# JingruiYu/FishBirdEyeVisualSLAM

Hardware: AMD Instinct MI355X
Metric: frames/s (extract+match+pose-opt), 1280x720+512x512 pair (higher is better)
Workload: dtype u8 (extract, Hamming) + f64 (pose optimisation); 1 GPU; configs[2]: 1280x720 front + 512x512 bird pair, HIP ORB extract + M3/M9 Hamming match + PoseOptimizationWithBird (~2k front + ~1k bird edges); nfeatures=2000, parallelism=replicas x1

## Files before the change

fishbirdeyevisualslam_amd/csrc/orb.hip:

```cpp
#include "fb_common.h"
#include "fb_fast_score.h"
#include "fb_primitives.h"

namespace {

constexpr int EDGE_THRESHOLD = 19;
constexpr int HALF_PATCH = 15;
constexpr int PATCH_SIZE = 31;
constexpr int BORDER = EDGE_THRESHOLD - 3;

__constant__ float c_pattern[1024] = {
#include "orb_pattern.inc"
};

struct LevelInfo {
  int w, h, pitch;
  long long off;
  int nCols, nRows, wCell, hCell, cellBase;
  int N;
  long long candBase;
  int candCap;
  int slotCap;
  int outBase, outCap;
  int nIni;
  float hX;
  float scale;
  int patchSize;
  long long boff;
};

struct OrbK {
  int nlevels, iniTh, minTh, totalCells, outStride, capOut;
  int kpStride;
  int fastTileBytes, fastMaxOut, fastMaxPix;
  int fastTP;
  int dbg;
  unsigned long long *timers;
  int cellBase[FB_MAX_LEVELS + 1];
  int grpBase[FB_MAX_LEVELS + 1];
  int totalGroups;
  long long pyrStride;
  long long blurStride;
  int blurStrips[FB_MAX_LEVELS + 1];
  long long candStride;
  int umax[16];
  LevelInfo L[FB_MAX_LEVELS];
};

struct ResizeTabs {
  const int *xofs;
  const short *ialpha;
  const int *yofs;
  const short *ibeta;
};

__device__ __forceinline__ int win_byte(uint32_t w0, uint32_t w1, uint32_t w2, uint32_t w3, int k) {
  const uint32_t lo = k & 8 ? w2 : w0, hi = k & 8 ? w3 : w1;
  const uint32_t w = k & 4 ? hi : lo;
  return (w >> (8 * (k & 3))) & 0xFF;
}

__global__ __launch_bounds__(256) void k_resize(const uint8_t *__restrict__ src0, long long srcImgStride, int sw,
                                                int sh, int spitch, uint8_t *__restrict__ dst0, long long dstImgStride,
                                                int dw, int dh, int dpitch, ResizeTabs tb) {
  const int b = blockIdx.z;
  const int dy = blockIdx.y * blockDim.y + threadIdx.y;
  const int dx4 = (blockIdx.x * blockDim.x + threadIdx.x) * 4;
  if (dy >= dh || dx4 >= dpitch) return;
  const uint8_t *src = src0 + (long long)b * srcImgStride;
  uint8_t *dst = dst0 + (long long)b * dstImgStride;
  int sy0 = tb.yofs[dy], sy1 = sy0 + 1;
  sy0 = sy0 >= 0 ? (sy0 < sh ? sy0 : sh - 1) : 0;
  sy1 = sy1 >= 0 ? (sy1 < sh ? sy1 : sh - 1) : 0;
  const int b0 = tb.ibeta[dy * 2], b1 = tb.ibeta[dy * 2 + 1];
  const uint8_t *r0p = src + (long long)sy0 * spitch, *r1p = src + (long long)sy1 * spitch;
  uint32_t packed = 0;
  const int dxl = min(dx4 + 3, dw - 1);
  const int sxa = dx4 < dw ? tb.xofs[dx4] : 0, sxb = dx4 < dw ? min(tb.xofs[dxl] + 1, sw - 1) : 0;
  const int a = sxa & ~3;
  const bool wide = ((reinterpret_cast<uintptr_t>(src) | (uintptr_t)spitch) & 3) == 0 && (sxb - a) < 16 && a + 16 <= spitch;
  if (wide) {
    const uint32_t *p0 = reinterpret_cast<const uint32_t *>(r0p + a), *p1 = reinterpret_cast<const uint32_t *>(r1p + a);
    const uint32_t u0 = p0[0], u1 = p0[1], u2 = p0[2], u3 = p0[3], v0 = p1[0], v1 = p1[1], v2 = p1[2], v3 = p1[3];
#pragma unroll
    for (int k = 0; k < 4; k++) {
// ... 504 lines not shown
          int oq = o - TP - 1;
          asm volatile("" : "+v"(oq));
          const uint8_t *q = &sc[oq] + TP + 1;
          const int sv = q[0];
          if (sv >= Tk) {
            const int mx = max(max(max(max((int)q[-1], (int)q[1]), (int)q[-tp - 1]), max((int)q[-tp], (int)q[-tp + 1])),
                               max(max((int)q[tp - 1], (int)q[tp]), (int)q[tp + 1]));
            keep = sv > mx;
            const int yy = o / tp, xx = o - yy * tp - ox;
            rec = (uint32_t)(x0 + xx) | ((uint32_t)(y0 + yy) << 12) | ((uint32_t)sv << 24);
          }
        }
        const unsigned long long m = __ballot(keep);
        if (keep) s_out[total + (int)__builtin_amdgcn_mbcnt_hi((uint32_t)(m >> 32), __builtin_amdgcn_mbcnt_lo((uint32_t)m, 0u))] = rec;
        total += __popcll(m);
      }
      if (pass == 0) { FAST_TICK(4) } else { FAST_TICK(7) }
      if (K.dbg == 3) { if (total == 12345) cand[0] = 1; return; }
      if (total == 0) continue;
      __syncthreads();
      uint32_t *out = cand + (long long)b * K.candStride + Lv.candBase + (long long)cell * Lv.slotCap;
#pragma unroll 1
      for (int i = lane; i < total; i += 64) out[i] = s_out[i];
      if (lane == 0) cellCount[(long long)b * K.totalCells + Lv.cellBase + cell] = total;
      if (pass == 0) { FAST_TICK(5) } else { FAST_TICK(8) }
      break;
    }
  };
  int ci = __builtin_amdgcn_readfirstlane(cFirst / Lv.nCols), cj = cFirst - ci * Lv.nCols;
  Geo g = geo(ci, cj);
  if (timed) { if (g.cw + g.ch + g.x0 + g.y0 == 123456789) cand[0] = 1; }
  FAST_TICK(9)
  if (g.ok && aligned) issue(g);
  for (int cell = cFirst; cell < cEnd; cell++) {
    const bool haveNext = cell + 1 < cEnd;
    if (haveNext) { cj++; if (cj == Lv.nCols) { cj = 0; ci++; } }
    const Geo gn = geo(ci, cj);
    if (g.ok) {
      stage(g);
      if (timed) { if (tile[lane] == 255 && sc[lane] == 7) cand[0] = 1; }
      FAST_TICK(0)
      __builtin_amdgcn_s_waitcnt(0x0F70);
      if (haveNext && gn.ok && aligned) issue(gn);
      FAST_TICK(1)
      process(g, cell);
      __syncthreads();
    } else if (haveNext && gn.ok && aligned) {
      issue(gn);
    }
    g = gn;
  }
  if (TIMED && timed && lane == 0) {
#pragma unroll
    for (int i = 0; i < 10; i++) atomicAdd(&K.timers[i], (unsigned long long)t_acc[i]);
    atomicAdd(&K.timers[10], (unsigned long long)(t_mark - t_start));
    atomicAdd(&K.timers[11], 1ull);
  }
#undef FAST_TICK
}

struct ONode {
  short x0, y0, x1, y1;
  int cnt;
};

__device__ __forceinline__ int quadrant(const ONode &n, int rx, int ry) {
  const int halfX = (int)ceilf((float)(n.x1 - n.x0) / 2), halfY = (int)ceilf((float)(n.y1 - n.y0) / 2);
  const int mx = n.x0 + halfX, my = n.y0 + halfY;
  return (rx < mx ? 0 : 1) + (ry < my ? 0 : 2);
}

__device__ __forceinline__ ONode child_of(const ONode &n, int q, int cnt) {
  const int halfX = (int)ceilf((float)(n.x1 - n.x0) / 2), halfY = (int)ceilf((float)(n.y1 - n.y0) / 2);
  const int mx = n.x0 + halfX, my = n.y0 + halfY;
  ONode c;
  c.x0 = (q & 1) ? mx : n.x0;
  c.x1 = (q & 1) ? n.x1 : mx;
  c.y0 = (q & 2) ? my : n.y0;
  c.y1 = (q & 2) ? n.y1 : my;
  c.cnt = cnt;
  return c;
}

template <int NT>
__global__ __launch_bounds__(NT) void k_octree(OrbK K, const uint32_t *__restrict__ cellCand, const int *__restrict__ cellCount,
                                                uint32_t *__restrict__ cand, int *__restrict__ candCount, uint16_t *__restrict__ nodeOf,
                                                uint32_t *__restrict__ lvlOut, int *__restrict__ lvlCount, int maxNodes) {
  extern __shared__ __attribute__((aligned(16))) uint8_t smem[];
  const int l = blockIdx.y, b = blockIdx.x, tid = threadIdx.x;
  const LevelInfo &Lv = K.L[l];
  const int M = maxNodes;
  ONode *listA = reinterpret_cast<ONode *>(smem);
  ONode *listB = listA + M;
  int *ccnt = reinterpret_cast<int *>(listB + M);
  unsigned short *cpos = reinterpret_cast<unsigned short *>(ccnt + 4 * M);
  unsigned short *npos = cpos + 4 * M;
  unsigned short *order = npos + M;
  unsigned char *split = reinterpret_cast<unsigned char *>(order + M);
  unsigned long long *best = reinterpret_cast<unsigned long long *>(smem + (((size_t)(split + M - smem)) + 7 & ~(size_t)7));
  __shared__ int s_w[NT / 64], s_S, s_nexp, s_jstar;
  uint32_t *cdw = cand + (long long)b * K.candStride + Lv.candBase;
  int n;
  {
    int *offs = reinterpret_cast<int *>(smem);
    const int ncell = Lv.nCols * Lv.nRows;
    const int *cc = cellCount + (long long)b * K.totalCells + Lv.cellBase;
    const uint32_t *sp = cellCand + (long long)b * K.candStride + Lv.candBase;
    int run = 0;
    for (int c0 = 0; c0 < ncell; c0 += NT) {
      const int c = c0 + tid;
      const int v = c < ncell ? cc[c] : 0;
      int tot;
      const int ex = fb::block_excl_scan<NT>(v, s_w, &tot);
      if (c < ncell) offs[c] = run + ex;
      run += tot;
      __syncthreads();
    }
    n = run;
    if (tid == 0) { offs[ncell] = n; candCount[b * K.nlevels + l] = n; }
    __syncthreads();
    for (int k0 = tid; k0 < n; k0 += NT * 4) {
      uint32_t val[4];
#pragma unroll
      for (int u = 0; u < 4; u++) {
        const int k = min(k0 + u * NT, n - 1);
        int lo = 0, hi = ncell;
        while (hi - lo > 1) {
          const int mid = (lo + hi) >> 1;
          if (offs[mid] <= k) lo = mid; else hi = mid;
        }
        val[u] = sp[(long long)lo * Lv.slotCap + (k - offs[lo])];
      }
#pragma unroll
      for (int u = 0; u < 4; u++)
        if (k0 + u * NT < n) cdw[k0 + u * NT] = val[u];
    }
    __threadfence_block();
    __syncthreads();
  }
  const uint32_t *cd = cdw;
  uint16_t *nof = nodeOf + (long long)b * K.candStride + Lv.candBase;
  int *outCount = lvlCount + b * K.nlevels + l;
  uint32_t *out = lvlOut + (long long)b * K.outStride + Lv.outBase;
  if (n == 0 || Lv.nIni < 1) { if (tid == 0) *outCount = 0; return; }
  const int N = Lv.N;
  const int Hh = Lv.h - 2 * BORDER;
  for (int i = tid; i < Lv.nIni; i += NT) {
    ONode nd;
    nd.x0 = (short)(int)(Lv.hX * (float)i);
    nd.x1 = (short)(int)(Lv.hX * (float)(i + 1));
    nd.y0 = 0; nd.y1 = (short)Hh; nd.cnt = 0;
    listB[i] = nd;
  }
  __syncthreads();
  for (int k = tid; k < n; k += NT) {
    const int rx = (int)(cd[k] & 0xFFF) - BORDER;
    int idx = (int)((float)rx / Lv.hX);
    idx = min(idx, Lv.nIni - 1);
    nof[k] = (uint16_t)idx;
    atomicAdd(&listB[idx].cnt, 1);
  }
  __syncthreads();
  if (tid == 0) {
    int S = 0;
    for (int i = 0; i < Lv.nIni; i++) {
      npos[i] = (unsigned short)S;
      if (listB[i].cnt > 0) listA[S++] = listB[i];
    }
    s_S = S;
  }
  __syncthreads();
  for (int k = tid; k < n; k += NT) nof[k] = npos[nof[k]];
  __syncthreads();
  ONode *cur = listA, *nxt = listB;
  int S = s_S;
  bool finalPhase = false;
  for (int guard = 0; guard < 64; guard++) {
    const int prevSize = S;
    for (int i = tid; i < 4 * S; i += NT) ccnt[i] = 0;
    __syncthreads();
    for (int k0 = tid; k0 < n; k0 += NT * 4) {
      int pk[4];
      uint32_t ck[4];
#pragma unroll
      for (int u = 0; u < 4; u++) { const int kk = min(k0 + u * NT, n - 1); pk[u] = nof[kk]; ck[u] = cd[kk]; }
#pragma unroll
      for (int u = 0; u < 4; u++) {
        if (k0 + u * NT >= n) break;
        const int p = pk[u];
        const ONode nd = cur[p];
        if (nd.cnt > 1) {
          const uint32_t c = ck[u];
          atomicAdd(&ccnt[4 * p + quadrant(nd, (int)(c & 0xFFF) - BORDER, (int)((c >> 12) & 0xFFF) - BORDER)], 1);
        }
      }
    }
    __syncthreads();
    if (!finalPhase) {
      for (int p = tid; p < S; p += NT) split[p] = cur[p].cnt > 1;
    } else {
      for (int p = tid; p < S; p += NT) {
        split[p] = 0;
        const int c = cur[p].cnt;
        if (c > 1) {
          int rank = 0;
          for (int j = 0; j < S; j++) {
            const int cj = cur[j].cnt;
            if (cj > 1 && (cj > c || (cj == c && j < p))) rank++;
          }
          order[rank] = (unsigned short)p;
        }
      }
      __syncthreads();
      if (tid == 0) {
        int sz = S, j = 0;
        const int C = s_nexp;
        for (; j < C; j++) {
          const int p = order[j];
          const int kk = (ccnt[4 * p] > 0) + (ccnt[4 * p + 1] > 0) + (ccnt[4 * p + 2] > 0) + (ccnt[4 * p + 3] > 0);
          sz += kk - 1;
          split[p] = 1;
          if (sz >= N) { j++; break; }
        }
        s_jstar = j;
      }
    }
    __syncthreads();
    const int per = (S + NT - 1) / NT;
    const int a0 = min(tid * per, S), a1 = min(a0 + per, S);
    int myKids = 0, myKeep = 0;
    if (!finalPhase) {
      for (int p = a0; p < a1; p++) {
        if (split[p]) myKids += (ccnt[4 * p] > 0) + (ccnt[4 * p + 1] > 0) + (ccnt[4 * p + 2] > 0) + (ccnt[4 * p + 3] > 0);
        else myKeep++;
      }
    } else {
      const int J = s_jstar;
      const int perj = (J + NT - 1) / NT;
      const int r0 = min(tid * perj, J), r1 = min(r0 + perj, J);
      for (int r = r0; r < r1; r++) {
        const int p = order[r];
        myKids += (ccnt[4 * p] > 0) + (ccnt[4 * p + 1] > 0) + (ccnt[4 * p + 2] > 0) + (ccnt[4 * p + 3] > 0);
      }
      for (int p = a0; p < a1; p++) if (!split[p]) myKeep++;
    }
    int totalKids, totalKeep;
    const int kidsBefore = fb::block_excl_scan<NT>(myKids, s_w, &totalKids);
    const int keepBefore = fb::block_excl_scan<NT>(myKeep, s_w, &totalKeep);
    {
      int ci = kidsBefore, kp = totalKids + keepBefore;
      if (!finalPhase) {
        for (int p = a0; p < a1; p++) {
          if (split[p]) {
            for (int q = 0; q < 4; q++)
              if (ccnt[4 * p + q] > 0) {
                const int pos = totalKids - 1 - ci++;
                cpos[4 * p + q] = (unsigned short)pos;
                nxt[pos] = child_of(cur[p], q, ccnt[4 * p + q]);
              }
          } else {
            npos[p] = (unsigned short)kp;
            nxt[kp++] = cur[p];
          }
        }
      } else {
        const int J = s_jstar;
        const int perj = (J + NT - 1) / NT;
        const int r0 = min(tid * perj, J), r1 = min(r0 + perj, J);
        for (int r = r0; r < r1; r++) {
          const int p = order[r];
          for (int q = 0; q < 4; q++)
            if (ccnt[4 * p + q] > 0) {
              const int pos = totalKids - 1 - ci++;
              cpos[4 * p + q] = (unsigned short)pos;
              nxt[pos] = child_of(cur[p], q, ccnt[4 * p + q]);
            }
        }
        for (int p = a0; p < a1; p++)
          if (!split[p]) { npos[p] = (unsigned short)kp; nxt[kp++] = cur[p]; }
      }
    }
    const int Snew = totalKids + totalKeep;
    __syncthreads();
    for (int k0 = tid; k0 < n; k0 += NT * 4) {
      int pk[4];
      uint32_t ck[4];
#pragma unroll
      for (int u = 0; u < 4; u++) { const int kk = min(k0 + u * NT, n - 1); pk[u] = nof[kk]; ck[u] = cd[kk]; }
#pragma unroll
      for (int u = 0; u < 4; u++) {
        const int k = k0 + u * NT;
        if (k >= n) break;
        const int p = pk[u];
        if (split[p]) {
          const uint32_t c = ck[u];
          nof[k] = cpos[4 * p + quadrant(cur[p], (int)(c & 0xFFF) - BORDER, (int)((c >> 12) & 0xFFF) - BORDER)];
        } else nof[k] = npos[p];
      }
    }
    int myExp = 0;
    {
      const int pern = (Snew + NT - 1) / NT;
      const int n0 = min(tid * pern, Snew), n1 = min(n0 + pern, Snew);
      for (int p = n0; p < n1; p++) myExp += (p < totalKids && nxt[p].cnt > 1);
    }
    int nToExpand;
    fb::block_excl_scan<NT>(myExp, s_w, &nToExpand);
    if (tid == 0) s_nexp = nToExpand;
    __syncthreads();
    ONode *t = cur; cur = nxt; nxt = t;
    S = Snew;
    if (S >= N || S == prevSize) break;
    if (!finalPhase) {
      if (S + nToExpand * 3 > N) finalPhase = true;
    }
  }
  for (int p = tid; p < S; p += NT) best[p] = 0ull;
  __syncthreads();
  for (int k0 = tid; k0 < n; k0 += NT * 4) {
    int pk[4];
    uint32_t ck[4];
#pragma unroll
    for (int u = 0; u < 4; u++) { const int kk = min(k0 + u * NT, n - 1); pk[u] = nof[kk]; ck[u] = cd[kk]; }
#pragma unroll
    for (int u = 0; u < 4; u++) {
    const int k = k0 + u * NT;
    if (k >= n) break;
    const uint32_t c = ck[u];
    const int x = c & 0xFFF, y = (c >> 12) & 0xFFF, r = c >> 24;
    const int cellI = (y - EDGE_THRESHOLD) / Lv.hCell, cellJ = (x - EDGE_THRESHOLD) / Lv.wCell;
    const int dwid = min(Lv.wCell, Lv.w - 2 * EDGE_THRESHOLD - cellJ * Lv.wCell);
    const int inCell = (y - EDGE_THRESHOLD - cellI * Lv.hCell) * dwid + (x - EDGE_THRESHOLD - cellJ * Lv.wCell);
    const unsigned orderKey = (unsigned)(cellI * Lv.nCols + cellJ) * 4096u + (unsigned)inCell;
    const unsigned long long key = ((unsigned long long)r << 56) | ((unsigned long long)(0xFFFFFFFFu - orderKey) << 24) | (unsigned)k;
    atomicMax(&best[pk[u]], key);
    }
  }
  __syncthreads();
  for (int p = tid; p < S; p += NT) out[p] = cd[(unsigned)(best[p] & 0xFFFFFFull)];
  if (tid == 0) *outCount = S;
}

constexpr int BLUR_ROWS = 32;

__device__ __forceinline__ int reflect101(int i, int n) {
  if (i < 0) i = -i;
  if (i >= n) i = 2 * n - 2 - i;
  return i;
}

__global__ __launch_bounds__(256) void k_blur(OrbK K, const uint8_t *__restrict__ img0, long long imgStride, int pitch0,
                                              const uint8_t *__restrict__ pyr, uint8_t *__restrict__ blur) {
  const int b = blockIdx.y;
  const int strip = __builtin_amdgcn_readfirstlane(blockIdx.x * 4 + (threadIdx.x >> 6));
  const int lane = threadIdx.x & 63;
  if (strip >= K.blurStrips[K.nlevels]) return;
  int l = 0;
  while (strip >= K.blurStrips[l + 1]) l++;
  const LevelInfo &L = K.L[l];
  const int w = L.w, h = L.h;
  const int sidx = strip - K.blurStrips[l];
  const int nsx = (w + 255) >> 8;
  const int sy = sidx / nsx, sx = sidx - sy * nsx;
  const int x0 = sx * 256 + lane * 4;
  const int y0 = sy * BLUR_ROWS;
  if (x0 >= w) return;
  const uint8_t *img;
  int pitch;
  if (l == 0) { img = img0 + (long long)b * imgStride; pitch = pitch0; }
  else { img = pyr + (long long)b * K.pyrStride + L.off; pitch = L.pitch; }
  uint8_t *out = blur + (long long)b * K.blurStride + L.boff;
  const bool edge = x0 < 4 || x0 + 8 > w;
  const int base = edge ? max(min(x0 - 4, w - 12), 0) : x0 - 4;
  uint32_t m1[3] = {0, 0, 0}, m2[3] = {0, 0, 0};
  if (edge) {
#pragma unroll
    for (int i = 0; i < 12; i++) {
      const int c = reflect101(min(x0 - 4 + i, w + 2), w);
      const int sidx8 = min(max(c - base, 0), 11);
      const uint32_t lo = sidx8 < 8 ? (uint32_t)sidx8 : 0x0cu, hi = sidx8 < 8 ? 0x0cu : (uint32_t)(sidx8 - 8);
      m1[i >> 2] |= lo << (8 * (i & 3));
      m2[i >> 2] |= hi << (8 * (i & 3));
    }
  }
  const bool anyEdge = __ballot(edge) != 0ull;
  const uint32_t WA = 18u | (34u << 8) | (49u << 16) | (55u << 24), WB = 49u | (34u << 8) | (18u << 16);
  uint32_t pairs[6][4];
  uint32_t prevh[4] = {0u, 0u, 0u, 0u};
  constexpr int BLUR_PF = 4;
  uint32_t q[BLUR_PF][3];
  auto loadRow = [&](int r, uint32_t (&dst)[3]) {
    const int ys = reflect101(min(y0 + r - 3, h + 2), h);
    const uint8_t *row = img + (uint32_t)__mul24(ys, pitch);
    const uint32_t *pw = reinterpret_cast<const uint32_t *>(row + base);
// ... 146 lines not shown
  };
  KP kpv[DESC_KPW];
#pragma unroll
  for (int j = 0; j < DESC_KPW; j++) {
    kpv[j] = decode(min(j, nmine - 1));
    if (j < nmine) issue(kpv[j], vb[j], vr[j]);
  }
#pragma unroll
  for (int j = 0; j < DESC_KPW; j++) {
    if (j >= nmine) break;
    const KP &cur = kpv[j];
    stage(cur, vb[j], vr[j]);
    int m10 = 0, m01 = 0;
    if (lane < 62) {
      const int r = lane >> 1, half = lane & 1;
      const int sb = cur.rox + (half ? 15 : 0);
      const uint32_t *rowd = rawp + r * DP_RAW_DW + (sb >> 2);
      const uint32_t sh = (uint32_t)(sb & 3);
      const uint32_t d0 = rowd[0], d1 = rowd[1], d2 = rowd[2], d3 = rowd[3], d4 = rowd[4];
      const uint32_t q0 = __builtin_amdgcn_alignbyte(d1, d0, sh), q1 = __builtin_amdgcn_alignbyte(d2, d1, sh);
      const uint32_t q2 = __builtin_amdgcn_alignbyte(d3, d2, sh), q3 = __builtin_amdgcn_alignbyte(d4, d3, sh);
      const uint4 W = angW, Km = angK;
      const uint32_t a10 = __builtin_amdgcn_udot4(q0, W.x, __builtin_amdgcn_udot4(q1, W.y, __builtin_amdgcn_udot4(q2, W.z, __builtin_amdgcn_udot4(q3, W.w, 0u, false), false), false), false);
      const uint32_t rs = __builtin_amdgcn_udot4(q0, Km.x, __builtin_amdgcn_udot4(q1, Km.y, __builtin_amdgcn_udot4(q2, Km.z, __builtin_amdgcn_udot4(q3, Km.w, 0u, false), false), false), false);
      m10 = half ? (int)a10 : -(int)a10;
      m01 = __mul24(r - 15, (int)rs);
    }
    m10 = fb::wave_sum(m10);
    m01 = fb::wave_sum(m01);
    if (K.dbg == 12) { if (m10 + m01 == 12345678 && (int)(pp[0].x + pp[1].y + pp[2].z + pp[3].w) == 77777) nOut[0] = 1; continue; }
    const float angle = fb_fast_atan2((float)m01, (float)m10);
    const float factorPI = 0x1.1df46ap-6f;
    float sa, ca;
    fb_sincos_f(angle * factorPI, &sa, &ca);
    const float a = ca, bb = sa;
    const uint8_t *centre = reinterpret_cast<const uint8_t *>(blp) + 18 * (DP_BL_DW * 4) + cur.box + 18;
    int nib = 0;
#pragma unroll
    for (int t = 0; t < 4; t++) {
      const float x0 = pp[t].x, y0 = pp[t].y, x1 = pp[t].z, y1 = pp[t].w;
      const int t0 = centre[__mul24(fb_cvround(x0 * bb + y0 * a), DP_BL_DW * 4) + fb_cvround(x0 * a - y0 * bb)];
      const int t1 = centre[__mul24(fb_cvround(x1 * bb + y1 * a), DP_BL_DW * 4) + fb_cvround(x1 * a - y1 * bb)];
      nib |= (t0 < t1) << t;
    }
    const int hi = __shfl_down(nib, 1, 64);
    const int byteVal = nib | (hi << 4);
    const int b1 = __shfl_down(byteVal, 2, 64), b2 = __shfl_down(byteVal, 4, 64), b3 = __shfl_down(byteVal, 6, 64);
    const uint32_t dw = (uint32_t)byteVal | ((uint32_t)b1 << 8) | ((uint32_t)b2 << 16) | ((uint32_t)b3 << 24);
    const long long o = (long long)b * K.kpStride + first + j;
    if ((lane & 7) == 0) reinterpret_cast<uint32_t *>(desc + o * 32)[lane >> 3] = dw;
    if (lane == 0) {
      fb_keypoint kp;
      kp.x = (float)cur.cx;
      kp.y = (float)cur.cy;
      if (cur.myl != 0) { kp.x *= cur.scale; kp.y *= cur.scale; }
      kp.size = (float)cur.patchSize;
      kp.angle = angle;
      kp.response = (float)cur.resp;
      kp.octave = cur.myl;
      kps[o] = kp;
    }
    __builtin_amdgcn_fence(__ATOMIC_RELEASE, "wavefront");
    __builtin_amdgcn_wave_barrier();
  }
}

}

struct fb_orb {
  fb_orb_params p;
  fb_orb_tables t;
  hipStream_t sideStream = nullptr;
  hipEvent_t evFork = nullptr, evJoin = nullptr;
  ~fb_orb() {
    if (evFork) (void)hipEventDestroy(evFork);
    if (evJoin) (void)hipEventDestroy(evJoin);
    if (sideStream) (void)hipStreamDestroy(sideStream);
  }
  int kpStride = 0;
  int w = 0, h = 0, batchCap = 0;
  OrbK K;
  int maxNodes = 0;
  size_t octreeLds = 0;
  fb::DevBuf pyr, blur, cand, cellCand, cellCount, nodeOf, counts, lvlOut, tabs, angTab, timers;
  ResizeTabs rt[FB_MAX_LEVELS];
  bool mergeOK[FB_MAX_LEVELS] = {};
  bool rowsOK[FB_MAX_LEVELS] = {};
  const uint8_t *lastImg = nullptr;
  long long lastImgStride = 0;
  int lastPitch0 = 0;
  fb::DevBuf ownedImg;
};

namespace {

void make_tables(const fb_orb_params &p, fb_orb_tables &t) {
  memset(&t, 0, sizeof(t));
  const int nl = p.nlevels;
  t.scale_factor[0] = 1.0f;
  t.level_sigma2[0] = 1.0f;
  for (int i = 1; i < nl; i++) {
    t.scale_factor[i] = t.scale_factor[i - 1] * p.scale_factor;
    t.level_sigma2[i] = t.scale_factor[i] * t.scale_factor[i];
  }
  for (int i = 0; i < nl; i++) {
    t.inv_scale_factor[i] = 1.0f / t.scale_factor[i];
    t.inv_level_sigma2[i] = 1.0f / t.level_sigma2[i];
  }
  float factor = 1.0f / p.scale_factor;
  float nDesired = p.nfeatures * (1 - factor) / (1 - (float)pow((double)factor, (double)nl));
  int sum = 0;
  for (int l = 0; l < nl - 1; l++) {
    t.features_per_level[l] = fb_cvround(nDesired);
    sum += t.features_per_level[l];
    nDesired *= factor;
  }
  t.features_per_level[nl - 1] = std::max(p.nfeatures - sum, 0);
  int umax[HALF_PATCH + 2] = {0};
  int v, v0;
  const int vmax = fb_cvfloor(HALF_PATCH * sqrtf(2.f) / 2 + 1);
  const int vmin = fb_cvceil(HALF_PATCH * sqrtf(2.f) / 2);
  const double hp2 = HALF_PATCH * HALF_PATCH;
  for (v = 0; v <= vmax; ++v) umax[v] = fb_cvround_d(sqrt(hp2 - v * v));
  for (v = HALF_PATCH, v0 = 0; v >= vmin; --v) {
    while (umax[v0] == umax[v0 + 1]) ++v0;
    umax[v] = v0;
    ++v0;
  }
  for (int i = 0; i <= HALF_PATCH; i++) t.umax[i] = umax[i];
}

int capacity_of(const fb_orb_params &p) { return p.nfeatures + 8 * p.nlevels; }

int prepare(fb_orb *o, int w, int h, int batch) {
  if (o->w == w && o->h == h && batch <= o->batchCap) return FB_OK;
  const fb_orb_params &p = o->p;
  OrbK &K = o->K;
  memset(&K, 0, sizeof(K));
  K.nlevels = p.nlevels;
  K.iniTh = p.ini_th_fast;
  K.minTh = p.min_th_fast;
  K.capOut = capacity_of(p);
  K.kpStride = o->kpStride > 0 ? o->kpStride : K.capOut;
  for (int i = 0; i < 16; i++) K.umax[i] = o->t.umax[i];
  long long pyrOff = 0, candOff = 0, blurOff = 0;
  int cells = 0, outOff = 0, maxNodes = 0, strips = 0;
  std::vector<int> xofs, yofs;
  std::vector<short> ialpha, ibeta;
  std::vector<size_t> tabOff(p.nlevels * 4, 0);
  std::vector<uint8_t> tabBytes;
  auto append = [&](const void *src, size_t n) {
    size_t off = (tabBytes.size() + 15) & ~(size_t)15;
    tabBytes.resize(off + n);
    memcpy(tabBytes.data() + off, src, n);
    return off;
  };
  int pw = w, ph = h;
  for (int l = 0; l < p.nlevels; l++) {
    LevelInfo &L = K.L[l];
    const float scale = o->t.inv_scale_factor[l];
    L.w = fb_cvround((float)w * scale);
    L.h = fb_cvround((float)h * scale);
    if (l == 0) { L.w = w; L.h = h; }
    if (L.w < 1 || L.h < 1) {
      fb::set_error("pyramid level %d of a %dx%d image is empty (scale factor %.3f, %d levels)", l, w, h, (double)p.scale_factor, p.nlevels);
      return FB_ERR_ARG;
// ... 36 lines not shown
    if (l > 0) {
      const int sw = pw, sh = ph, dwd = L.w, dhd = L.h;
      const double inv_scale_x = (double)dwd / sw, inv_scale_y = (double)dhd / sh;
      const double scale_x = 1. / inv_scale_x, scale_y = 1. / inv_scale_y;
      xofs.assign(dwd, 0); ialpha.assign(dwd * 2, 0); yofs.assign(dhd, 0); ibeta.assign(dhd * 2, 0);
      for (int dx = 0; dx < dwd; dx++) {
        float fx = (float)((dx + 0.5) * scale_x - 0.5);
        int sx = fb_cvfloor(fx);
        fx -= sx;
        if (sx < 0) { fx = 0; sx = 0; }
        if (sx >= sw - 1) { fx = 0; sx = sw - 1; }
        xofs[dx] = sx;
        ialpha[dx * 2] = (short)fb_cvround((1.f - fx) * 2048.f);
        ialpha[dx * 2 + 1] = (short)fb_cvround(fx * 2048.f);
      }
      for (int dy = 0; dy < dhd; dy++) {
        float fy = (float)((dy + 0.5) * scale_y - 0.5);
        int sy = fb_cvfloor(fy);
        fy -= sy;
        yofs[dy] = sy;
        ibeta[dy * 2] = (short)fb_cvround((1.f - fy) * 2048.f);
        ibeta[dy * 2 + 1] = (short)fb_cvround(fy * 2048.f);
      }
      bool ok = true;
      for (int dx4 = 0; dx4 < dwd; dx4 += 4) {
        const int last = xofs[std::min(dx4 + 3, dwd - 1)] + 1;
        ok = ok && (last - (xofs[dx4] & ~3)) <= 11 && (last - xofs[dx4]) <= 7;
      }
      o->rowsOK[l] = ok;
      {
        bool okm = ok;
        for (int y0 = 0; y0 < dhd && okm; y0 += RM_ROWS) {
          const int y1 = std::min(y0 + RM_ROWS, dhd) - 1;
          okm = yofs[y0] >= 0 && yofs[y1] + 1 - yofs[y0] <= RM_SRC - 1;
          for (int y = y0; y < y1 && okm; y++) okm = yofs[y + 1] > yofs[y];
        }
        o->mergeOK[l] = okm;
      }
      tabOff[l * 4 + 0] = append(xofs.data(), xofs.size() * 4);
      tabOff[l * 4 + 1] = append(ialpha.data(), ialpha.size() * 2);
      tabOff[l * 4 + 2] = append(yofs.data(), yofs.size() * 4);
      tabOff[l * 4 + 3] = append(ibeta.data(), ibeta.size() * 2);
    }
    pw = L.w; ph = L.h;
  }
  K.totalCells = cells;
  {
    int gsum = 0;
    for (int l = 0; l <= FB_MAX_LEVELS; l++) {
      K.grpBase[l] = gsum;
      if (l < p.nlevels) gsum += (K.L[l].nCols * K.L[l].nRows + FAST_CPW - 1) / FAST_CPW;
    }
    K.totalGroups = gsum;
  }
  for (int l = 0; l <= FB_MAX_LEVELS; l++) K.cellBase[l] = l < p.nlevels ? K.L[l].cellBase : cells;
  K.dbg = getenv("FB_FAST_DBG") ? atoi(getenv("FB_FAST_DBG")) : 0;
  {
    int tileB = 0, maxOut = 0, maxPix = 0, tpNeed = 0;
    for (int l = 0; l < p.nlevels; l++) {
      const LevelInfo &L = K.L[l];
      if (L.nCols * L.nRows == 0) continue;
      const int tpMax = (L.wCell + 6 + 3 + 3) & ~3, chMax = L.hCell + 6;
      tpNeed = std::max(tpNeed, tpMax);
      tileB = std::max(tileB, chMax);
      maxOut = std::max(maxOut, ((L.wCell + 1) / 2) * ((L.hCell + 1) / 2));
      maxPix = std::max(maxPix, L.wCell * L.hCell);
    }
    K.fastTP = tpNeed <= 44 ? 44 : tpNeed <= 56 ? 56 : FAST_MAX_TILE;
    K.fastTileBytes = (std::max(K.fastTP * tileB, 4 * ((maxOut + 3) & ~3)) + 15) & ~15;
    K.fastTileBytes = std::max(K.fastTileBytes, (21 * K.fastTP + 15) & ~15);
    K.fastMaxOut = (maxOut + 3) & ~3;
    K.fastMaxPix = (maxPix + 7) & ~7;
  }
  K.pyrStride = (pyrOff + 255) & ~255ll;
  K.blurStride = (blurOff + 255) & ~255ll;
  for (int l = p.nlevels; l <= FB_MAX_LEVELS; l++) K.blurStrips[l] = strips;
  K.candStride = candOff;
  K.outStride = outOff;
  o->maxNodes = maxNodes;
  const size_t M = maxNodes;
  size_t lds = 2 * M * sizeof(ONode) + 4 * M * 4 + 4 * M * 2 + M * 2 + M * 2 + M;
  lds = ((lds + 7) & ~(size_t)7) + M * 8 + 16;
  {
    size_t maxCells = 0;
    for (int l = 0; l < p.nlevels; l++) maxCells = std::max(maxCells, (size_t)K.L[l].nCols * K.L[l].nRows);
    lds = std::max(lds, (maxCells + 1) * 4 + 16);
  }
  if (lds > 160 * 1024 - 512) { fb::set_error("nfeatures too large for the LDS quadtree (%zu B)", lds); return FB_ERR_CAPACITY; }
  o->octreeLds = lds;
  FB_TRY(o->tabs.upload(tabBytes.data(), tabBytes.size()));
  for (int l = 1; l < p.nlevels; l++) {
    const uint8_t *base = o->tabs.as<uint8_t>();
    o->rt[l].xofs = reinterpret_cast<const int *>(base + tabOff[l * 4 + 0]);
    o->rt[l].ialpha = reinterpret_cast<const short *>(base + tabOff[l * 4 + 1]);
    o->rt[l].yofs = reinterpret_cast<const int *>(base + tabOff[l * 4 + 2]);
    o->rt[l].ibeta = reinterpret_cast<const short *>(base + tabOff[l * 4 + 3]);
  }
  const size_t B = batch;
  {
    std::vector<uint32_t> tab(64 * 8, 0);
    for (int lane = 0; lane < 62; lane++) {
      const int v = (lane >> 1) - 15, half = lane & 1, dmax = K.umax[v < 0 ? -v : v];
      for (int j = 0; j < 16; j++) {
        const int au = half ? j : 15 - j;
        const bool inc = au <= dmax && (half || au != 0);
        if (!inc) continue;
        tab[lane * 8 + (j >> 2)] |= (uint32_t)au << (8 * (j & 3));
        tab[lane * 8 + 4 + (j >> 2)] |= 1u << (8 * (j & 3));
      }
    }
    FB_TRY(o->angTab.upload(tab.data(), tab.size() * 4));
  }
  FB_TRY(o->pyr.alloc(B * K.pyrStride + 256));
  FB_TRY(o->blur.alloc(B * K.blurStride + 256));
  FB_TRY(o->cand.alloc(B * K.candStride * 4 + 16));
  FB_TRY(o->cellCand.alloc(B * K.candStride * 4 + 16));
  FB_TRY(o->cellCount.alloc(B * (size_t)K.totalCells * 4 + 16));
  FB_TRY(o->nodeOf.alloc(B * K.candStride * 2 + 16));
  FB_TRY(o->counts.alloc(B * p.nlevels * 4 * 2));
  FB_TRY(o->timers.alloc(FB_ORB_TIMER_WORDS * 8));
  FB_HIP(hipMemset(o->timers.p, 0, FB_ORB_TIMER_WORDS * 8));
  K.timers = o->timers.as<unsigned long long>();
  FB_TRY(o->lvlOut.alloc(B * K.outStride * 4 + 16));
  o->w = w; o->h = h; o->batchCap = batch;
  return FB_OK;
}

}

extern "C" {

int fb_orb_capacity(const fb_orb_params *params) {
  if (!params) return FB_ERR_ARG;
  return capacity_of(*params);
}

int fb_orb_set_output_stride(fb_orb *h, int kp_stride) {
  FB_ARG(h && (kp_stride == 0 || kp_stride >= capacity_of(h->p)));
  h->kpStride = kp_stride;
  h->K.kpStride = kp_stride > 0 ? kp_stride : capacity_of(h->p);
  return FB_OK;
}

int fb_orb_create(const fb_orb_params *params, fb_orb **out) {
  FB_ARG(params && out);
  FB_ARG(params->nlevels >= 1 && params->nlevels <= FB_MAX_LEVELS);
  FB_ARG(params->nfeatures >= 1 && params->nfeatures <= 60000);
  FB_ARG(params->scale_factor > 1.0f);
  FB_ARG(params->min_th_fast >= 1 && params->ini_th_fast >= params->min_th_fast && params->ini_th_fast <= 254);
  fb_orb *o = new fb_orb();
  o->p = *params;
  make_tables(o->p, o->t);
  *out = o;
  return FB_OK;
}

void fb_orb_destroy(fb_orb *h) { delete h; }

int fb_orb_get_tables(const fb_orb *h, fb_orb_tables *out) {
  FB_ARG(h && out);
  *out = h->t;
  return FB_OK;
}

int fb_orb_extract_batch_dev(fb_orb *o, const uint8_t *d_images, int batch, int width, int height, int stride,
                             size_t image_stride, fb_keypoint *d_keypoints, uint8_t *d_descriptors, int32_t *d_n,
                             void *stream) {
  FB_TRY(fb::check_device());
  FB_ARG(o && d_images && d_keypoints && d_descriptors && d_n);
  FB_ARG(batch >= 1 && width >= 2 * EDGE_THRESHOLD + 7 && height >= 2 * EDGE_THRESHOLD + 7 && stride >= width);
  FB_TRY(prepare(o, width, height, batch));
  hipStream_t s = fb::as_stream(stream);
  const OrbK &K = o->K;
  const int nl = K.nlevels;
  int *candCount = o->counts.as<int>();
  int *lvlCount = candCount + (size_t)o->batchCap * nl;
  FB_HIP(hipMemsetAsync(o->cellCount.p, 0, (size_t)batch * K.totalCells * 4, s));
  for (int l = 1; l < nl; l++) {
    const LevelInfo &D = K.L[l], &S = K.L[l - 1];
    const uint8_t *src = (l == 1) ? d_images : o->pyr.as<uint8_t>() + S.off;
    const long long sstr = (l == 1) ? (long long)image_stride : K.pyrStride;
    const int spitch = (l == 1) ? stride : S.pitch;
    dim3 blk(64, 4), grd((D.pitch / 4 + 63) / 64, (D.h + 3) / 4, batch);
    fb::ProfScope prof_(fb::P_RESIZE, s);
    const bool rows = o->rowsOK[l] && spitch >= 12 && ((reinterpret_cast<uintptr_t>(src) | (uintptr_t)spitch | (uintptr_t)sstr) & 3) == 0;
    if (rows && o->mergeOK[l]) {
      dim3 grdM((D.pitch / 4 + 63) / 64, (D.h + 4 * RM_ROWS - 1) / (4 * RM_ROWS), batch);
      k_resize_merge<<<grdM, blk, 0, s>>>(src, sstr, S.w, S.h, spitch, o->pyr.as<uint8_t>() + D.off, K.pyrStride, D.w, D.h, D.pitch, o->rt[l]);
    } else if (rows) {
      dim3 grdR((D.pitch / 4 + 63) / 64, (D.h + 4 * RESIZE_ROWS - 1) / (4 * RESIZE_ROWS), batch);
      k_resize_rows<<<grdR, blk, 0, s>>>(src, sstr, S.w, S.h, spitch, o->pyr.as<uint8_t>() + D.off, K.pyrStride, D.w, D.h, D.pitch, o->rt[l]);
    } else {
      k_resize<<<grd, blk, 0, s>>>(src, sstr, S.w, S.h, spitch, o->pyr.as<uint8_t>() + D.off, K.pyrStride, D.w, D.h, D.pitch, o->rt[l]);
    }
  }
  if (K.totalCells > 0) {
    fb::ProfScope prof_(K.fastTP == 44 ? fb::P_FAST : K.fastTP == 56 ? fb::P_FAST56 : fb::P_FAST72, s);
    const dim3 grdF((K.totalGroups + 7) / 8 * 8, batch);
    const size_t ldsF = (size_t)2 * K.fastTileBytes + 2 * K.fastMaxPix;
#define FAST_LAUNCH(TP_) { if (K.dbg == 20) k_fast<TP_, true><<<grdF, 64, ldsF, s>>>(K, d_images, (long long)image_stride, stride, o->pyr.as<uint8_t>(), o->cellCand.as<uint32_t>(), o->cellCount.as<int>()); \
                          else k_fast<TP_, false><<<grdF, 64, ldsF, s>>>(K, d_images, (long long)image_stride, stride, o->pyr.as<uint8_t>(), o->cellCand.as<uint32_t>(), o->cellCount.as<int>()); }
    if (K.fastTP == 44)
      FAST_LAUNCH(44)
    else if (K.fastTP == 56)
      FAST_LAUNCH(56)
    else
      FAST_LAUNCH(FAST_MAX_TILE)
#undef FAST_LAUNCH
  }
  static const int sideMin = [] {
    const char* e = getenv("FB_ORB_SIDE_MIN");
    return e ? atoi(e) : 64;
  }();
  const bool fork = batch >= sideMin && !(fb::g_prof_on && fb::g_prof_only < 0);
  hipStream_t sBlur = s;
  if (fork) {
    if (!o->sideStream) {
      FB_HIP(hipStreamCreateWithFlags(&o->sideStream, hipStreamNonBlocking));
      FB_HIP(hipEventCreateWithFlags(&o->evFork, hipEventDisableTiming));
      FB_HIP(hipEventCreateWithFlags(&o->evJoin, hipEventDisableTiming));
    }
    sBlur = o->sideStream;
    FB_HIP(hipEventRecord(o->evFork, s));
    FB_HIP(hipStreamWaitEvent(sBlur, o->evFork, 0));
  }
#ifndef FB_ORB_ABLATE_BLUR
  {
    fb::ProfScope prof_(fb::P_BLUR, sBlur);
    k_blur<<<dim3((K.blurStrips[nl] + 3) / 4, batch), 256, 0, sBlur>>>(K, d_images, (long long)image_stride, stride, o->pyr.as<uint8_t>(),
                                                                        o->blur.as<uint8_t>());
  }
#endif
  if (fork) FB_HIP(hipEventRecord(o->evJoin, sBlur));
  static const int octWideMax = getenv("FB_OCT_WIDE_MAX") ? atoi(getenv("FB_OCT_WIDE_MAX")) : 512;
  const bool octWide = nl * batch <= octWideMax;
  FB_HIP(hipFuncSetAttribute(octWide ? reinterpret_cast<const void *>(k_octree<1024>) : reinterpret_cast<const void *>(k_octree<256>), hipFuncAttributeMaxDynamicSharedMemorySize, (int)o->octreeLds));
  {
  fb::ProfScope prof_(fb::P_OCTREE, s);
  if (octWide)
    k_octree<1024><<<dim3(batch, nl), 1024, o->octreeLds, s>>>(K, o->cellCand.as<uint32_t>(), o->cellCount.as<int>(), o->cand.as<uint32_t>(), candCount, o->nodeOf.as<uint16_t>(),
                                                          o->lvlOut.as<uint32_t>(), lvlCount, o->maxNodes);
  else
    k_octree<256><<<dim3(batch, nl), 256, o->octreeLds, s>>>(K, o->cellCand.as<uint32_t>(), o->cellCount.as<int>(), o->cand.as<uint32_t>(), candCount, o->nodeOf.as<uint16_t>(),
                                                         o->lvlOut.as<uint32_t>(), lvlCount, o->maxNodes);
  }
  if (fork) FB_HIP(hipStreamWaitEvent(s, o->evJoin, 0));
  {
  fb::ProfScope prof_(fb::P_DESCRIBE, s);
  k_describe<<<dim3(((K.capOut + DESC_WPB * DESC_KPW - 1) / (DESC_WPB * DESC_KPW) + 7) / 8 * 8, batch), 64 * DESC_WPB, 0, s>>>(K, d_images, (long long)image_stride, stride, o->pyr.as<uint8_t>(),
                                                   o->blur.as<uint8_t>(), o->angTab.as<uint4>(), o->lvlOut.as<uint32_t>(), lvlCount, d_keypoints,
                                                   d_descriptors, d_n);
  }
  FB_HIP(hipGetLastError());
  o->lastImg = d_images;
  o->lastImgStride = (long long)image_stride;
  o->lastPitch0 = stride;
  return FB_OK;
}

int fb_orb_extract(fb_orb *o, const uint8_t *image, int width, int height, int stride, fb_keypoint *keypoints,
                   uint8_t *descriptors, int32_t *n_out) {
  FB_TRY(fb::check_device());
  FB_ARG(o && n_out);
  if (!image || width <= 0 || height <= 0) return FB_OK;
  FB_ARG(keypoints && descriptors && stride >= width);
  const int cap = capacity_of(o->p);
  const size_t imgBytes = (size_t)stride * height, kpBytes = (size_t)cap * sizeof(fb_keypoint), dBytes = (size_t)cap * 32;
  const size_t oN = 0, oK = 256, oD = oK + ((kpBytes + 255) & ~(size_t)255), oC = oD + ((dBytes + 255) & ~(size_t)255), outBytes = oC + 256;
  const size_t imgArea = fb::Stager::up256(imgBytes);
  uint8_t *pin = static_cast<uint8_t *>(fb::pinned_scratch(imgArea + outBytes));
  if (!pin) return FB_ERR_HIP;
  fb::DevBuf dout;
  FB_TRY(dout.alloc(outBytes));
  if (o->ownedImg.bytes < imgBytes || !o->ownedImg.p) FB_TRY(o->ownedImg.alloc(imgBytes));
  memcpy(pin, image, imgBytes);
  struct SyncOnError {
    bool armed = true;
    ~SyncOnError() { if (armed) { (void)hipStreamSynchronize(nullptr); (void)hipGetLastError(); } }
  } guard;
  FB_HIP(hipMemcpyAsync(o->ownedImg.p, pin, imgBytes, hipMemcpyHostToDevice, nullptr));
  uint8_t *dbase = dout.as<uint8_t>();
  const int keepStride = o->kpStride;
  if (keepStride) FB_TRY(fb_orb_set_output_stride(o, 0));
  const int rc = fb_orb_extract_batch_dev(o, o->ownedImg.as<uint8_t>(), 1, width, height, stride, imgBytes, reinterpret_cast<fb_keypoint *>(dbase + oK),
                                          dbase + oD, reinterpret_cast<int32_t *>(dbase + oN), nullptr);
  if (keepStride) (void)fb_orb_set_output_stride(o, keepStride);
  FB_TRY(rc);
  uint8_t *pout = pin + imgArea;
  FB_HIP(hipMemcpyAsync(pout, dbase, oC, hipMemcpyDeviceToHost, nullptr));
  FB_HIP(hipMemcpyAsync(pout + oC, o->counts.as<int>() + (size_t)o->batchCap * o->p.nlevels, (size_t)o->p.nlevels * 4, hipMemcpyDeviceToHost, nullptr));
  FB_HIP(hipStreamSynchronize(nullptr));
  guard.armed = false;
  memcpy(n_out, pout + oN, 4);
  {
    const int *lc = reinterpret_cast<const int *>(pout + oC);
    int total = 0;
    for (int l = 0; l < o->p.nlevels; l++) total += lc[l];
    if (total > cap) {
      fb::set_error("keypoint capacity exceeded: the quadtree kept %d key points, fb_orb_capacity() is %d", total, cap);
      return FB_ERR_CAPACITY;
    }
  }
  memcpy(keypoints, pout + oK, (size_t)*n_out * sizeof(fb_keypoint));
  memcpy(descriptors, pout + oD, (size_t)*n_out * 32);
  return FB_OK;
}

int fb_orb_debug_timers(fb_orb *o, uint64_t *dst16) {
  FB_TRY(fb::check_device());
  FB_ARG(o && dst16 && o->timers.p);
  FB_HIP(hipDeviceSynchronize());
  FB_HIP(hipMemcpy(dst16, o->timers.p, 16 * 8, hipMemcpyDeviceToHost));
  FB_HIP(hipMemset(o->timers.p, 0, 16 * 8));
  return FB_OK;
}

#ifdef FB_FAST_LISTHIST
extern "C" int fb_orb_debug_list_hist(fb_orb *o, uint64_t *dst128) {
  FB_TRY(fb::check_device());
  FB_ARG(o && dst128 && o->timers.p);
  FB_HIP(hipDeviceSynchronize());
  FB_HIP(hipMemcpy(dst128, o->timers.as<unsigned long long>() + 16, 128 * 8, hipMemcpyDeviceToHost));
  FB_HIP(hipMemset(o->timers.as<unsigned long long>() + 16, 0, 128 * 8));
  return FB_OK;
}
#endif

// ... 40 lines not shown
```

Before: 70600 frames/s.

## Fuse octree quadrant counting into compaction and child-assignment passes

Removes the separate per-iteration pass over all candidates that counted quadrant occupancy. The counts for the initial nodes are now accumulated while candidates are gathered, and later iterations accumulate child quadrant counts during the reassignment pass. Empty initial nodes are kept in the list and skipped, which drops the serial thread-0 compaction. The per-call hipFuncSetAttribute is also moved to setup behind a per-device cache. The cost is extra LDS for the initial counts and more complex bookkeeping for empty nodes.

```diff
diff --git a/fishbirdeyevisualslam_amd/csrc/orb.hip b/fishbirdeyevisualslam_amd/csrc/orb.hip
--- a/fishbirdeyevisualslam_amd/csrc/orb.hip
+++ b/fishbirdeyevisualslam_amd/csrc/orb.hip
@@ -1,6 +1,8 @@
 #include "fb_common.h"
 #include "fb_fast_score.h"
 #include "fb_primitives.h"
+
+#include <mutex>
 
 namespace {
 
@@ -671,10 +673,18 @@
   return c;
 }
 
+__device__ __forceinline__ ONode ini_node(const LevelInfo &Lv, int i, int cnt) {
+  ONode nd;
+  nd.x0 = (short)(int)(Lv.hX * (float)i);
+  nd.x1 = (short)(int)(Lv.hX * (float)(i + 1));
+  nd.y0 = 0; nd.y1 = (short)(Lv.h - 2 * BORDER); nd.cnt = cnt;
+  return nd;
+}
+
 template <int NT>
 __global__ __launch_bounds__(NT) void k_octree(OrbK K, const uint32_t *__restrict__ cellCand, const int *__restrict__ cellCount,
                                                 uint32_t *__restrict__ cand, int *__restrict__ candCount, uint16_t *__restrict__ nodeOf,
-                                                uint32_t *__restrict__ lvlOut, int *__restrict__ lvlCount, int maxNodes) {
+                                                uint32_t *__restrict__ lvlOut, int *__restrict__ lvlCount, int maxNodes, int iniOff) {
   extern __shared__ __attribute__((aligned(16))) uint8_t smem[];
   const int l = blockIdx.y, b = blockIdx.x, tid = threadIdx.x;
   const LevelInfo &Lv = K.L[l];
@@ -687,18 +697,22 @@
   unsigned short *order = npos + M;
   unsigned char *split = reinterpret_cast<unsigned char *>(order + M);
   unsigned long long *best = reinterpret_cast<unsigned long long *>(smem + (((size_t)(split + M - smem)) + 7 & ~(size_t)7));
-  __shared__ int s_w[NT / 64], s_S, s_nexp, s_jstar;
+  int *cc0 = reinterpret_cast<int *>(smem + iniOff);
+  __shared__ int s_w[NT / 64], s_nexp, s_jstar;
   uint32_t *cdw = cand + (long long)b * K.candStride + Lv.candBase;
+  uint16_t *nof = nodeOf + (long long)b * K.candStride + Lv.candBase;
+  const int nIni = Lv.nIni;
   int n;
   {
     int *offs = reinterpret_cast<int *>(smem);
     const int ncell = Lv.nCols * Lv.nRows;
-    const int *cc = cellCount + (long long)b * K.totalCells + Lv.cellBase;
+    const int *cellN = cellCount + (long long)b * K.totalCells + Lv.cellBase;
     const uint32_t *sp = cellCand + (long long)b * K.candStride + Lv.candBase;
     int run = 0;
+    for (int i = tid; i < 4 * nIni; i += NT) cc0[i] = 0;
     for (int c0 = 0; c0 < ncell; c0 += NT) {
       const int c = c0 + tid;
-      const int v = c < ncell ? cc[c] : 0;
+      const int v = c < ncell ? cellN[c] : 0;
       int tot;
       const int ex = fb::block_excl_scan<NT>(v, s_w, &tot);
       if (c < ncell) offs[c] = run + ex;
@@ -721,70 +735,41 @@
         val[u] = sp[(long long)lo * Lv.slotCap + (k - offs[lo])];
       }
 #pragma unroll
-      for (int u = 0; u < 4; u++)
-        if (k0 + u * NT < n) cdw[k0 + u * NT] = val[u];
+      for (int u = 0; u < 4; u++) {
+        const int k = k0 + u * NT;
+        if (k >= n) break;
+        cdw[k] = val[u];
+        if (nIni >= 1) {
+          const int rx = (int)(val[u] & 0xFFF) - BORDER, ry = (int)((val[u] >> 12) & 0xFFF) - BORDER;
+          const int idx = min((int)((float)rx / Lv.hX), nIni - 1);
+          nof[k] = (uint16_t)idx;
+          atomicAdd(&cc0[4 * idx + quadrant(ini_node(Lv, idx, 0), rx, ry)], 1);
+        }
+      }
     }
     __threadfence_block();
     __syncthreads();
   }
   const uint32_t *cd = cdw;
-  uint16_t *nof = nodeOf + (long long)b * K.candStride + Lv.candBase;
   int *outCount = lvlCount + b * K.nlevels + l;
   uint32_t *out = lvlOut + (long long)b * K.outStride + Lv.outBase;
-  if (n == 0 || Lv.nIni < 1) { if (tid == 0) *outCount = 0; return; }
+  if (n == 0 || nIni < 1) { if (tid == 0) *outCount = 0; return; }
   const int N = Lv.N;
-  const int Hh = Lv.h - 2 * BORDER;
-  for (int i = tid; i < Lv.nIni; i += NT) {
-    ONode nd;
-    nd.x0 = (short)(int)(Lv.hX * (float)i);
-    nd.x1 = (short)(int)(Lv.hX * (float)(i + 1));
-    nd.y0 = 0; nd.y1 = (short)Hh; nd.cnt = 0;
-    listB[i] = nd;
-  }
-  __syncthreads();
-  for (int k = tid; k < n; k += NT) {
-    const int rx = (int)(cd[k] & 0xFFF) - BORDER;
-    int idx = (int)((float)rx / Lv.hX);
-    idx = min(idx, Lv.nIni - 1);
-    nof[k] = (uint16_t)idx;
-    atomicAdd(&listB[idx].cnt, 1);
-  }
-  __syncthreads();
-  if (tid == 0) {
-    int S = 0;
-    for (int i = 0; i < Lv.nIni; i++) {
-      npos[i] = (unsigned short)S;
-      if (listB[i].cnt > 0) listA[S++] = listB[i];
-    }
-    s_S = S;
-  }
-  __syncthreads();
-  for (int k = tid; k < n; k += NT) nof[k] = npos[nof[k]];
-  __syncthreads();
   ONode *cur = listA, *nxt = listB;
-  int S = s_S;
+  const int *cc = cc0;
+  int S = nIni, prevSize = 0;
+  {
+    int mine = 0;
+    for (int i = tid; i < nIni; i += NT) {
+      const int c = cc0[4 * i] + cc0[4 * i + 1] + cc0[4 * i + 2] + cc0[4 * i + 3];
+      cur[i] = ini_node(Lv, i, c);
+      mine += c > 0;
+    }
+    prevSize = fb::block_sum<NT>(mine, s_w);
+  }
   bool finalPhase = false;
   for (int guard = 0; guard < 64; guard++) {
-    const int prevSize = S;
-    for (int i = tid; i < 4 * S; i += NT) ccnt[i] = 0;
-    __syncthreads();
-    for (int k0 = tid; k0 < n; k0 += NT * 4) {
-      int pk[4];
-      uint32_t ck[4];
-#pragma unroll
-      for (int u = 0; u < 4; u++) { const int kk = min(k0 + u * NT, n - 1); pk[u] = nof[kk]; ck[u] = cd[kk]; }
-#pragma unroll
-      for (int u = 0; u < 4; u++) {
-        if (k0 + u * NT >= n) break;
-        const int p = pk[u];
-        const ONode nd = cur[p];
-        if (nd.cnt > 1) {
-          const uint32_t c = ck[u];
-          atomicAdd(&ccnt[4 * p + quadrant(nd, (int)(c & 0xFFF) - BORDER, (int)((c >> 12) & 0xFFF) - BORDER)], 1);
-        }
-      }
-    }
-    __syncthreads();
+    if (guard > 0) prevSize = S;
     if (!finalPhase) {
       for (int p = tid; p < S; p += NT) split[p] = cur[p].cnt > 1;
     } else {
@@ -806,7 +791,7 @@
         const int C = s_nexp;
         for (; j < C; j++) {
           const int p = order[j];
-          const int kk = (ccnt[4 * p] > 0) + (ccnt[4 * p + 1] > 0) + (ccnt[4 * p + 2] > 0) + (ccnt[4 * p + 3] > 0);
+          const int kk = (cc[4 * p] > 0) + (cc[4 * p + 1] > 0) + (cc[4 * p + 2] > 0) + (cc[4 * p + 3] > 0);
           sz += kk - 1;
           split[p] = 1;
           if (sz >= N) { j++; break; }
@@ -820,8 +805,8 @@
     int myKids = 0, myKeep = 0;
     if (!finalPhase) {
       for (int p = a0; p < a1; p++) {
-        if (split[p]) myKids += (ccnt[4 * p] > 0) + (ccnt[4 * p + 1] > 0) + (ccnt[4 * p + 2] > 0) + (ccnt[4 * p + 3] > 0);
-        else myKeep++;
+        if (split[p]) myKids += (cc[4 * p] > 0) + (cc[4 * p + 1] > 0) + (cc[4 * p + 2] > 0) + (cc[4 * p + 3] > 0);
+        else if (cur[p].cnt > 0) myKeep++;
       }
     } else {
       const int J = s_jstar;
@@ -829,9 +814,9 @@
       const int r0 = min(tid * perj, J), r1 = min(r0 + perj, J);
       for (int r = r0; r < r1; r++) {
         const int p = order[r];
-        myKids += (ccnt[4 * p] > 0) + (ccnt[4 * p + 1] > 0) + (ccnt[4 * p + 2] > 0) + (ccnt[4 * p + 3] > 0);
-      }
-      for (int p = a0; p < a1; p++) if (!split[p]) myKeep++;
+        myKids += (cc[4 * p] > 0) + (cc[4 * p + 1] > 0) + (cc[4 * p + 2] > 0) + (cc[4 * p + 3] > 0);
+      }
+      for (int p = a0; p < a1; p++) if (!split[p] && cur[p].cnt > 0) myKeep++;
     }
     int totalKids, totalKeep;
     const int kidsBefore = fb::block_excl_scan<NT>(myKids, s_w, &totalKids);
@@ -842,12 +827,12 @@
         for (int p = a0; p < a1; p++) {
           if (split[p]) {
             for (int q = 0; q < 4; q++)
-              if (ccnt[4 * p + q] > 0) {
+              if (cc[4 * p + q] > 0) {
                 const int pos = totalKids - 1 - ci++;
                 cpos[4 * p + q] = (unsigned short)pos;
-                nxt[pos] = child_of(cur[p], q, ccnt[4 * p + q]);
+                nxt[pos] = child_of(cur[p], q, cc[4 * p + q]);
               }
-          } else {
+          } else if (cur[p].cnt > 0) {
             npos[p] = (unsigned short)kp;
             nxt[kp++] = cur[p];
           }
@@ -859,17 +844,19 @@
         for (int r = r0; r < r1; r++) {
           const int p = order[r];
           for (int q = 0; q < 4; q++)
-            if (ccnt[4 * p + q] > 0) {
+            if (cc[4 * p + q] > 0) {
               const int pos = totalKids - 1 - ci++;
               cpos[4 * p + q] = (unsigned short)pos;
-              nxt[pos] = child_of(cur[p], q, ccnt[4 * p + q]);
+              nxt[pos] = child_of(cur[p], q, cc[4 * p + q]);
             }
         }
         for (int p = a0; p < a1; p++)
-          if (!split[p]) { npos[p] = (unsigned short)kp; nxt[kp++] = cur[p]; }
+          if (!split[p] && cur[p].cnt > 0) { npos[p] = (unsigned short)kp; nxt[kp++] = cur[p]; }
       }
     }
     const int Snew = totalKids + totalKeep;
+    __syncthreads();
+    for (int i = tid; i < 4 * totalKids; i += NT) ccnt[i] = 0;
     __syncthreads();
     for (int k0 = tid; k0 < n; k0 += NT * 4) {
       int pk[4];
@@ -883,7 +870,11 @@
         const int p = pk[u];
         if (split[p]) {
           const uint32_t c = ck[u];
-          nof[k] = cpos[4 * p + quadrant(cur[p], (int)(c & 0xFFF) - BORDER, (int)((c >> 12) & 0xFFF) - BORDER)];
+          const int rx = (int)(c & 0xFFF) - BORDER, ry = (int)((c >> 12) & 0xFFF) - BORDER;
+          const int np = cpos[4 * p + quadrant(cur[p], rx, ry)];
+          const ONode ch = nxt[np];
+          if (ch.cnt > 1) atomicAdd(&ccnt[4 * np + quadrant(ch, rx, ry)], 1);
+          nof[k] = (uint16_t)np;
         } else nof[k] = npos[p];
       }
     }
@@ -899,6 +890,7 @@
     __syncthreads();
     ONode *t = cur; cur = nxt; nxt = t;
     S = Snew;
+    cc = ccnt;
     if (S >= N || S == prevSize) break;
     if (!finalPhase) {
       if (S + nToExpand * 3 > N) finalPhase = true;
@@ -1211,6 +1203,7 @@
   OrbK K;
   int maxNodes = 0;
   size_t octreeLds = 0;
+  int octIniOff = 0;
   fb::DevBuf pyr, blur, cand, cellCand, cellCount, nodeOf, counts, lvlOut, tabs, angTab, timers;
   ResizeTabs rt[FB_MAX_LEVELS];
   bool mergeOK[FB_MAX_LEVELS] = {};
@@ -1413,12 +1406,33 @@
   size_t lds = 2 * M * sizeof(ONode) + 4 * M * 4 + 4 * M * 2 + M * 2 + M * 2 + M;
   lds = ((lds + 7) & ~(size_t)7) + M * 8 + 16;
   {
-    size_t maxCells = 0;
-    for (int l = 0; l < p.nlevels; l++) maxCells = std::max(maxCells, (size_t)K.L[l].nCols * K.L[l].nRows);
-    lds = std::max(lds, (maxCells + 1) * 4 + 16);
+    size_t maxCells = 0, maxIni = 0;
+    for (int l = 0; l < p.nlevels; l++) {
+      maxCells = std::max(maxCells, (size_t)K.L[l].nCols * K.L[l].nRows);
+      maxIni = std::max(maxIni, (size_t)std::max(K.L[l].nIni, 0));
+    }
+    const size_t offsBytes = (maxCells + 1) * 4 + 16, ccntOff = 2 * M * sizeof(ONode);
+    size_t iniOff = ccntOff;
+    if (offsBytes > ccntOff) {
+      iniOff = (std::max(offsBytes, lds) + 15) & ~(size_t)15;
+      lds = iniOff + 16 * maxIni + 16;
+    }
+    o->octIniOff = (int)iniOff;
   }
   if (lds > 160 * 1024 - 512) { fb::set_error("nfeatures too large for the LDS quadtree (%zu B)", lds); return FB_ERR_CAPACITY; }
   o->octreeLds = lds;
+  {
+    static std::mutex mu;
+    static size_t granted[64] = {};
+    int dev = 0;
+    FB_HIP(hipGetDevice(&dev));
+    std::lock_guard<std::mutex> lock(mu);
+    if (dev < 0 || dev >= 64 || lds > granted[dev]) {
+      FB_HIP(hipFuncSetAttribute(reinterpret_cast<const void *>(k_octree<1024>), hipFuncAttributeMaxDynamicSharedMemorySize, (int)lds));
+      FB_HIP(hipFuncSetAttribute(reinterpret_cast<const void *>(k_octree<256>), hipFuncAttributeMaxDynamicSharedMemorySize, (int)lds));
+      if (dev >= 0 && dev < 64) granted[dev] = lds;
+    }
+  }
   FB_TRY(o->tabs.upload(tabBytes.data(), tabBytes.size()));
   for (int l = 1; l < p.nlevels; l++) {
     const uint8_t *base = o->tabs.as<uint8_t>();
@@ -1565,15 +1579,14 @@
   if (fork) FB_HIP(hipEventRecord(o->evJoin, sBlur));
   static const int octWideMax = getenv("FB_OCT_WIDE_MAX") ? atoi(getenv("FB_OCT_WIDE_MAX")) : 512;
   const bool octWide = nl * batch <= octWideMax;
-  FB_HIP(hipFuncSetAttribute(octWide ? reinterpret_cast<const void *>(k_octree<1024>) : reinterpret_cast<const void *>(k_octree<256>), hipFuncAttributeMaxDynamicSharedMemorySize, (int)o->octreeLds));
   {
   fb::ProfScope prof_(fb::P_OCTREE, s);
   if (octWide)
     k_octree<1024><<<dim3(batch, nl), 1024, o->octreeLds, s>>>(K, o->cellCand.as<uint32_t>(), o->cellCount.as<int>(), o->cand.as<uint32_t>(), candCount, o->nodeOf.as<uint16_t>(),
-                                                          o->lvlOut.as<uint32_t>(), lvlCount, o->maxNodes);
+                                                          o->lvlOut.as<uint32_t>(), lvlCount, o->maxNodes, o->octIniOff);
   else
     k_octree<256><<<dim3(batch, nl), 256, o->octreeLds, s>>>(K, o->cellCand.as<uint32_t>(), o->cellCount.as<int>(), o->cand.as<uint32_t>(), candCount, o->nodeOf.as<uint16_t>(),
-                                                         o->lvlOut.as<uint32_t>(), lvlCount, o->maxNodes);
+                                                         o->lvlOut.as<uint32_t>(), lvlCount, o->maxNodes, o->octIniOff);
   }
   if (fork) FB_HIP(hipStreamWaitEvent(s, o->evJoin, 0));
   {
```

New measurement: 71010 frames/s, median of 6. No clear change (+0.6%).
